# tudoroancea/ihm2

Measured on AMD Instinct MI355X. Metric: NMPC RTI solves/s (batch), N=40, nx=8 (6-DOF bicycle), fkin6, higher is better.
Workload: dtype f64

## Files before the change

ihm2_amd/csrc/kernels_qp.hip:

```cpp
#include <cstring>

#include "ihm2mpc_internal.h"
#include "device_steps.hpp"
#include "sqp_body.hpp"
#include "irk_body.hpp"
#include "riccati_mfma.hpp"
#include "sens_body.hpp"
#include "qp_lds.hpp"
#include "qp_mrows.hpp"
#include "qp_reduce.hpp"
#include "qp_div.hpp"
#include "qp_catalogue.hpp"
#include "wave_sync.hpp"

using namespace ihm2;

namespace {

#define INF_BOUND 1e20
#ifndef RIC_RING
#define RIC_RING 4
#endif
#ifndef SWEEP_RING
#define SWEEP_RING 4
#endif
#define SWEEP_DL ((SWEEP_RING >= 8) ? 4 : 2)

__device__ __forceinline__ bool fin(double v) { return fabs(v) < INF_BOUND; }
__device__ __forceinline__ int here(int v) { asm volatile("" : "+v"(v)); return v; }

template <typename OP>
__device__ __forceinline__ double wave_reduce(double v, OP op)
{
    v = op(v, dpp_mov<0xB1>(v));
    v = op(v, dpp_mov<0x4E>(v));
    v = op(v, dpp_mov<0x141>(v));
    v = op(v, dpp_mov<0x128>(v));
    int lo = __double2loint(v), hi = __double2hiint(v);
    auto a16 = __builtin_amdgcn_permlane16_swap(lo, lo, false, false);
    auto b16 = __builtin_amdgcn_permlane16_swap(hi, hi, false, false);
    v = op(__hiloint2double(b16[0], a16[0]), __hiloint2double(b16[1], a16[1]));
    lo = __double2loint(v); hi = __double2hiint(v);
    auto a32 = __builtin_amdgcn_permlane32_swap(lo, lo, false, false);
    auto b32 = __builtin_amdgcn_permlane32_swap(hi, hi, false, false);
    return op(__hiloint2double(b32[0], a32[0]), __hiloint2double(b32[1], a32[1]));
}
__device__ __forceinline__ double nanmax(double a, double b) { return (a != a || b != b) ? NAN : fmax(a, b); }
__device__ __forceinline__ double wave_max(double v) { return wave_reduce(v, [](double a, double b) { return fmax(a, b); }); }
__device__ __forceinline__ double wave_min(double v) { return wave_reduce(v, [](double a, double b) { return fmin(a, b); }); }
__device__ __forceinline__ double wave_sum(double v) { return wave_reduce(v, [](double a, double b) { return a + b; }); }
__device__ __forceinline__ double wave_nanmax(double v) { return wave_reduce(v, [](double a, double b) { return nanmax(a, b); }); }
__device__ __forceinline__ void norm_max(double &res, bool &bad, double v) { bad |= v != v; res = fmax(res, v); }

__device__ __forceinline__ double sum8(double v)
{
    v += dpp_mov<0xB1>(v);
    v += dpp_mov<0x4E>(v);
    v += dpp_mov<0x141>(v);
    return v;
}

// ... 128 lines not shown
#undef LEN
#define HS(k, i, l) (HL ? Hl[(((k) == N) ? 100 : 0) + (i) * 10 + (l)] : ((k) == N ? HsT : Hs0 + (UNI ? 0 : (k)) * 100)[(i) * 10 + (l)])
#define CDV(k, r, j) (CL ? CDl[(r) * 10 + (j)] : a.CD[((k) * 2 + (r)) * 10 + (j)])

    auto blk_reduce = [&](double v, auto op) -> double {
        v = wave_reduce(v, op);
        if (NW > 1) {
            __syncthreads();
            if (lane == 0) tile[wv] = v;
            __syncthreads();
            v = tile[0];
#pragma unroll
            for (int w = 1; w < NW; w++) v = op(v, tile[w]);
        }
        return v;
    };
    auto blk_max = [&](double v) { return blk_reduce(v, [](double x, double y) { return fmax(x, y); }); };
    auto blk_min = [&](double v) { return blk_reduce(v, [](double x, double y) { return fmin(x, y); }); };
    auto blk_sum = [&](double v) { return blk_reduce(v, [](double x, double y) { return x + y; }); };
    auto blk_nanmax = [&](double v) { return blk_reduce(v, [](double x, double y) { return nanmax(x, y); }); };

    const double *xb = a.x + (size_t)b * NS * 8;
    const double *ub = a.u + (size_t)b * N * 2;
    const double *linb = a.lin + (size_t)b * N * LIN_REC;
    double *gb = a.g + (size_t)b * NS * 10;
    double *rgb = a.rg + (size_t)b * NS * 10;
    double *Pg = a.P + (size_t)b * NS * 64;
    double *Mg = a.M + (size_t)b * N * 64;
    double *pib = a.pi + (size_t)b * NS * 8;
    double *lamb = a.lam + (size_t)b * NS * 28;
    double *slkb = a.slk + (size_t)b * NS * 28;
    double *lamab = ALAT ? a.lam_a + (size_t)b * NS * 2 : nullptr;
    double *slkab = ALAT ? a.slk_a + (size_t)b * NS * 2 : nullptr;
    auto alat_slot = [](int j) -> int { return (j == 3) ? 0 : (j == 4) ? 1 : (j == 6) ? 2 : (j == 7) ? 3 : -1; };

    if (HL) for (int e = tid; e < 200; e += NT) Hl[e] = (e < 100) ? Hs0[e] : HsT[e - 100];
    if (CL && tid < 20) CDl[tid] = a.CD[tid];
    if (UNI) BSYNC();
    bool h_sparse = false;
    if (HL) {
        int cnt = 0;
        if (tid < 20) {
#pragma unroll
            for (int l = 0; l < 10; l++) {
                const double v = Hl[tid * 10 + l];
                if (v != 0.0) { if (cnt < 3) { spv[tid * 3 + cnt] = v; spc[tid * 3 + cnt] = l; } cnt++; }
            }
            for (int q = cnt; q < 3; q++) { spv[tid * 3 + q] = 0.0; spc[tid * 3 + q] = 0; }
        }
        h_sparse = __ballot(cnt > 3) == 0ull;
        if (NW > 1) h_sparse = blk_max((wv == 0 && !h_sparse) ? 1.0 : 0.0) == 0.0;
        BSYNC();
    }
    double sg = 1.0, sb = 1.0, r_stat = 0.0, r_eq = 0.0;
    double w_R = 0.0, w_L = 0.0;
    if (PATH) {
        const int trk = a.track_id[b];
        w_R = a.widths[trk * 2 + 0]; w_L = a.widths[trk * 2 + 1];
        for (int k = tid; k < NS; k += NT) {
            const double psi = xb[k * 8 + 2], sgn = (psi > 0.0) - (psi < 0.0);
            const double dfoot = -0.5 * a.car_L * cos(fabs(psi)) * sgn, dlat = -0.5 * a.car_W * sin(psi);
            hc[k * 2 + 0] = (k >= 1) ? dfoot + dlat : 0.0;
            hc[k * 2 + 1] = (k >= 1) ? -dfoot + dlat : 0.0;
            if (ALAT) {
                double g4[4];
                alat_eval(xb[k * 8 + 3], xb[k * 8 + 4], xb[k * 8 + 6], xb[k * 8 + 7], g4);
#pragma unroll
                for (int q = 0; q < 4; q++) ha[k * 4 + q] = (k >= 1 && k < N) ? g4[q] : 0.0;
            }
        }
        BSYNC();
    }
    for (int e = tid; e < NS * 10; e += NT) {
        const int k = e / 10, j = e % 10;
        double acc = 0.0;
#pragma unroll
        for (int l = 0; l < 8; l++) acc = fma(HS(k, j, l), xb[k * 8 + l], acc);
        if (k < N) {
            acc = fma(HS(k, j, 8), ub[k * 2 + 0], acc);
            acc = fma(HS(k, j, 9), ub[k * 2 + 1], acc);
            const double *yr = a.yref + ((size_t)b * N + k) * 12;
#pragma unroll
            for (int l = 0; l < 12; l++) acc = fma(-Gy0[((UNI ? 0 : k) * 10 + j) * 12 + l], yr[l], acc);
        } else {
            const double *yr = a.yref_e + (size_t)b * 8;
#pragma unroll
            for (int l = 0; l < 8; l++) acc = fma(-GyT[j * 12 + l], yr[l], acc);
        }
        gb[e] = acc;
        const bool counted = !((k == 0 && j < 8) || (k == N && j >= 8));
        if (j < 8 || k < N) sg = fmax(sg, fabs(acc));
        if (!want_res) continue;
        double st = acc;
        if (k < N) {
            const double *rec = linb + (size_t)k * LIN_REC;
#pragma unroll
            for (int l = 0; l < 8; l++) st = fma((j < 8) ? rec[l * 8 + j] : rec[64 + l * 2 + (j - 8)], pib[(k + 1) * 8 + l], st);
        }
        if (j < 8) st -= pib[k * 8 + j];
        st -= lamb[k * 28 + j] - lamb[k * 28 + 14 + j];
        if (k < N) {
            st = fma(-CDV(k, 0, j), lamb[k * 28 + 10] - lamb[k * 28 + 24], st);
            st = fma(-CDV(k, 1, j), lamb[k * 28 + 11] - lamb[k * 28 + 25], st);
        }
        if (PATH && (j == 1 || j == 2)) {
            const double l12 = lamb[k * 28 + 12] - lamb[k * 28 + 26], l13 = lamb[k * 28 + 13] - lamb[k * 28 + 27];
// ... 68 lines not shown
            if (r < NSOFT) { const size_t po = (size_t)b * a.sl_bs + a.nslots_can; const double *zp = a.slot_lb + po, *Zp = a.slot_ub + po; so_zw[r < NSOFT ? r : 0] = zp[s]; so_Zw[r < NSOFT ? r : 0] = Zp[s]; soft = Zp[s] >= 0.0; }
#define LAM_IN(up) ((ALAT && c == 14) ? lamab[k * 2 + (up)] : lamb[k * 28 + 14 * (up) + c])
            if (fin(lb)) { s_dl[r] = lb - cz; if (want_res && !soft) { r_ineq = fmax(r_ineq, s_dl[r]); r_comp = fmax(r_comp, fabs(LAM_IN(0) * s_dl[r])); } }
            if (fin(ubd)) { s_du[r] = ubd - cz; if (want_res && !soft) { r_ineq = fmax(r_ineq, -s_du[r]); r_comp = fmax(r_comp, fabs(LAM_IN(1) * s_du[r])); } }
#undef LAM_IN
            if (ONE_SIDED(r) && fin(ubd)) { s_sg[r < NSOFT ? r : 0] = -1.0; s_dl[r] = -s_du[r]; }
        }
    }
    if (want_res) {
        if constexpr (FULL != 0) wave_max4(lane, r_stat, r_eq, r_ineq, r_comp);
        else { r_stat = blk_max(r_stat); r_eq = blk_max(r_eq); r_ineq = blk_max(r_ineq); r_comp = blk_max(r_comp); }
    }
    if (want_res && tid == 0) {
        double *rs = a.res + (size_t)b * 4;
        rs[0] = r_stat; rs[1] = r_eq; rs[2] = r_ineq; rs[3] = r_comp;
    }

    const double tol_g = a.tol * sg, tol_b = a.tol * sb, tol_d = a.tol * sb, tol_m = a.tol * sg;
    const double mu_floor = 0.1 * tol_m;
    const double mu0 = a.mu0 * sg;
    const double inv_m = (a.m_act > 0) ? 1.0 / a.m_act : 0.0;

    auto row_dot = [&](int kc, const double *v) -> double {
        const int k = kc / NCK, c = kc % NCK;
        if (c < 10) return v[k * 10 + c];
        if (ALAT && c == 14) return ha[k * 4] * v[k * 10 + 3] + ha[k * 4 + 1] * v[k * 10 + 4] + ha[k * 4 + 2] * v[k * 10 + 6] + ha[k * 4 + 3] * v[k * 10 + 7];
        if (PATH && c >= 12) return (c == 12) ? v[k * 10 + 1] + hc[k * 2] * v[k * 10 + 2] : -v[k * 10 + 1] + hc[k * 2 + 1] * v[k * 10 + 2];
        double acc = 0.0;
#pragma unroll
        for (int j = 0; j < 10; j++) acc = fma(CDV(k, c - 10, j), v[k * 10 + j], acc);
        return acc;
    };
    auto row_dot_full = [&](int r, const double *v) -> double {
        const int pk = here(s_kc[r]);
        return *reinterpret_cast<const double *>(reinterpret_cast<const char *>(pk < 0 ? tile : v) + ((pk >> 16) & 0x3fff));
    };
    static_assert(FULL == 0 || qp_general_rows_inside(qp_lds(NF > 0 ? NF : 2, CLS), NF > 0 ? NF : 2), "the general rows of a phase leave the transpose tile");
    auto general_rows = [&](const double *v) {
        for (int e0 = tid; e0 < 2 * N; e0 += 2 * NT) {
            const bool two = e0 + NT < 2 * N;
            const double *cd = CDl + (e0 & 1) * 10, *v0 = v + (e0 >> 1) * 10, *v1 = v + ((two ? e0 + NT : e0) >> 1) * 10;
            double c[10], p[10], q[10];
#pragma unroll
            for (int j = 0; j < 10; j++) { c[j] = cd[j]; p[j] = v0[j]; q[j] = v1[j]; }
            double acc0 = 0.0, acc1 = 0.0;
#pragma unroll
            for (int j = 0; j < 10; j++) { acc0 = fma(c[j], p[j], acc0); acc1 = fma(c[j], q[j], acc1); }
            tile[e0] = acc0;
            if (two) tile[e0 + NT] = acc1;
        }
        BSYNC();
    };

    for (int e = tid; e < NS * 10; e += NT) z[e] = (e < 8) ? a.x0[(size_t)b * 8 + e] - xb[e] : 0.0;
    for (int e = tid; e < NS * 8; e += NT) pi[e] = 0.0;
    if (FULL) for (int e = tid; e < NS * NCK; e += NT) { cf[e] = 0.0; gam[e] = 0.0; }
    BSYNC();
    if constexpr (FULL != 0) general_rows(z);
#pragma unroll
    for (int r = 0; r < NSLOT; r++) {
        if (NO_SLOT(r)) continue;
        const double rz = ROW_DOT(r, z);
        const bool al = HAS_L(r), au = HAS_U(r);
        double tau_c = a.tau0;
        if (al && au) tau_c = fmin(a.tau0, 0.25 * (s_du[r] - s_dl[r]));
        if (IS_SOFT(r)) {
            const double slack = al ? rz - s_dl[r] : s_du[r] - rz;
            const double s0 = fmax(a.tau0, a.tau0 - slack);
            so_s[r < NSOFT ? r : 0] = s0;
            so_ls[r < NSOFT ? r : 0] = mu0 / s0;
            if (al) { t_l[r] = slack + s0; lam_l[r] = mu0 / t_l[r]; } else { t_u[r] = slack + s0; lam_u[r] = mu0 / t_u[r]; }
            continue;
        }
        if (al) { t_l[r] = fmax(rz - s_dl[r], tau_c); lam_l[r] = mu0 / t_l[r]; }
        if (au) { t_u[r] = fmax(s_du[r] - rz, tau_c); lam_u[r] = mu0 / t_u[r]; }
    }

    int qstatus = 1, it = 0;
    bool exact_mode = false;
    double res_g = 0, res_b = 0, res_d = 0, res_m = 0, mu = 0;
    double fol_g = 0.0, fol_b = 0.0;
    double rd_l[NSLOT], rd_u[NSLOT], dlam_l[NSLOT], dlam_u[NSLOT], dt_l[NSLOT], dt_u[NSLOT];
    double pa_l[NSLOT], pa_u[NSLOT];
    for (it = 0;; it++) {
        bool exact = (it == 0) || exact_mode, finished = false;
        auto multipliers_to_cf = [&]() {
            if (!FULL) {
                for (int e = tid; e < NS * NCK; e += NT) cf[e] = 0.0;
                BSYNC();
            }
#pragma unroll
            for (int r = 0; r < NSLOT; r++) {
                if (NO_SLOT(r)) continue;
                const bool al = HAS_L(r), au = HAS_U(r);
                SLOT_ACC(SLOT_AT(cf, r), ROW_SIGN(r, (al ? lam_l[r] : 0.0) - (au ? lam_u[r] : 0.0)));
            }
            BSYNC();
        };
        if (LEAN != 0) { if (exact) multipliers_to_cf(); }
        else {
            for (int e = tid; e < NS * NCK; e += NT) cf[e] = 0.0;
            BSYNC();
        }
        double mu_acc = 0.0, res_gs = 0.0;
        res_d = 0.0; res_m = 0.0;
        double lane_d = 0.0, lane_m = 0.0;
        bool bad_d = false, bad_m = false, bad_gs = false;
        if constexpr (FULL != 0) general_rows(z);
#pragma unroll
        for (int r = 0; r < NSLOT; r++) {
            rd_l[r] = rd_u[r] = 0.0;
            if (NO_SLOT(r)) continue;
            const double rz = ROW_DOT(r, z);
            const bool al = HAS_L(r), au = HAS_U(r);
            const double sv = IS_SOFT(r) ? so_s[r < NSOFT ? r : 0] : 0.0;
            double pl = 0.0, pu = 0.0;
            if constexpr (FULL != 0) {
                rd_l[r] = rz - t_l[r] - s_dl[r] + sv; pl = __dmul_rn(lam_l[r], t_l[r]); norm_max(lane_m, bad_m, fabs(pl));
                rd_u[r] = s_du[r] - rz - t_u[r] + sv; pu = __dmul_rn(lam_u[r], t_u[r]); norm_max(lane_m, bad_m, fabs(pu));
            } else {
            if (al) { rd_l[r] = rz - t_l[r] - s_dl[r] + sv; pl = __dmul_rn(lam_l[r], t_l[r]); res_m = nanmax(res_m, fabs(pl)); }
            if (au) { rd_u[r] = s_du[r] - rz - t_u[r] + sv; pu = __dmul_rn(lam_u[r], t_u[r]); res_m = nanmax(res_m, fabs(pu)); }
            }
            mu_acc = __dadd_rn(mu_acc, __dadd_rn(pl, pu));
            if constexpr (FULL != 0) { bad_d |= __builtin_isunordered(rd_l[r], rd_u[r]); lane_d = fmax(lane_d, fmax(fabs(rd_l[r]), fabs(rd_u[r]))); }
            else
            res_d = nanmax(res_d, nanmax(fabs(rd_l[r]), fabs(rd_u[r])));
            if (IS_SOFT(r)) {
                const int q = r < NSOFT ? r : 0;
                so_rs[q] = so_Zw[q] * so_s[q] + so_zw[q] - (al ? lam_l[r] : lam_u[r]) - so_ls[q];
                if constexpr (FULL != 0) {
                    norm_max(res_gs, bad_gs, fabs(so_rs[q]));
                    mu_acc += so_ls[q] * so_s[q]; norm_max(lane_m, bad_m, fabs(so_ls[q] * so_s[q]));
                } else {
                res_gs = nanmax(res_gs, fabs(so_rs[q]));
                mu_acc += so_ls[q] * so_s[q]; res_m = nanmax(res_m, fabs(so_ls[q] * so_s[q]));
                }
            }
            if (LEAN == 0) SLOT_ACC(SLOT_AT(cf, r), ROW_SIGN(r, (al ? lam_l[r] : 0.0) - (au ? lam_u[r] : 0.0)));
        }
        if constexpr (NW > 1) {
#pragma unroll
            for (int r = 0; r < NSLOT; r++) {
                const int sidx = tid + NT * r;
                if (sidx >= a.nslots_can) continue;
                const bool on = s_kc[r] >= 0;
                gam[sidx] = __dadd_rn((on && fin(s_dl[r])) ? __dmul_rn(lam_l[r], t_l[r]) : 0.0, (on && fin(s_du[r])) ? __dmul_rn(lam_u[r], t_u[r]) : 0.0);
            }
            __syncthreads();
            mu_acc = 0.0;
            for (int sidx = lane; sidx < a.nslots_can; sidx += 64) mu_acc = __dadd_rn(mu_acc, gam[sidx]);
            __syncthreads();
        }
        if (LEAN == 0) BSYNC();
        for (int rpass = 0; rpass < 2; rpass++) {
            if (exact) {
                for (int e = tid; e < NS * 10; e += NT) {
                    const int k = e / 10, j = e % 10;
                    double acc = gb[e];
                    if (HL && h_sparse) {
                        const int row = ((k == N) ? 10 : 0) + j;
#pragma unroll
                        for (int q = 0; q < 3; q++) acc = fma(spv[row * 3 + q], z[k * 10 + spc[row * 3 + q]], acc);
                    } else {
#pragma unroll
                        for (int l = 0; l < 10; l++) acc = fma(HS(k, j, l), z[k * 10 + l], acc);
                    }
                    if (k < N) {
                        acc = fma(-CDV(k, 0, j), cf[k * NCK + 10], acc);
                        acc = fma(-CDV(k, 1, j), cf[k * NCK + 11], acc);
                    }
                    if (j < 8) acc -= pi[k * 8 + j];
                    acc -= cf[k * NCK + j];
                    if (PATH && (j == 1 || j == 2)) {
                        const double l12 = cf[k * NCK + 12], l13 = cf[k * NCK + 13];
                        acc -= (j == 1) ? l12 - l13 : hc[k * 2] * l12 + hc[k * 2 + 1] * l13;
                    }
                    if (ALAT && alat_slot(j) >= 0) acc -= ha[k * 4 + alat_slot(j)] * cf[k * NCK + 14];
                    gt[e] = acc;
                }
                BSYNC();
                dyn_residual<4, NT>(N, tid, const_cast<double *>(linb), z, pi, gt, rb, LIN_REC);
                BSYNC();
            }
            res_g = 0.0; res_b = 0.0;
            if (exact || LEAN == 0) {
                for (int e = tid; e < NS * 10; e += NT) {
                    const int k = e / 10, j = e % 10;
                    double v = gt[e];
                    if ((k == 0 && j < 8) || (k == N && j >= 8)) { v = 0.0; gt[e] = 0.0; }
                    if (exact) rgb[e] = v;
                    res_g = nanmax(res_g, fabs(v));
                }
                for (int e = tid; e < N * 8; e += NT) res_b = nanmax(res_b, fabs(rb[e]));
            } else { res_g = fol_g; res_b = fol_b; }
            if constexpr (FULL != 0) {
                const bool nan_g = wave_any(res_g != res_g || bad_gs), nan_b = wave_any(res_b != res_b), nan_d = wave_any(bad_d), nan_m = wave_any(bad_m);
                res_g = fmax(res_g, res_gs);
                res_d = lane_d; res_m = lane_m;
                wave_max4(lane, res_g, res_b, res_d, res_m);
                mu = wave_sum(mu_acc) * inv_m;
                res_g = nan_g ? NAN : res_g; res_b = nan_b ? NAN : res_b; res_d = nan_d ? NAN : res_d; res_m = nan_m ? NAN : res_m;
            } else {
            res_g = nanmax(res_g, res_gs);
            res_g = blk_nanmax(res_g); res_b = blk_nanmax(res_b);
            if (rpass == 0) { res_d = blk_nanmax(res_d); res_m = blk_nanmax(res_m); mu = ((NW == 1) ? blk_sum(mu_acc) : wave_sum(mu_acc)) * inv_m; }
            }
            if (!(res_g == res_g) || !(res_b == res_b) || !(res_d == res_d) || !(res_m == res_m)) { qstatus = (it == 0) ? 3 : 4; finished = true; break; }
            const bool conv = res_g <= tol_g && res_b <= tol_b && res_d <= tol_d && res_m <= tol_m;
            if (conv && exact) { qstatus = 0; finished = true; break; }
            if ((conv || it >= a.iter_max) && !exact) {
                exact = true; exact_mode = true;
                if (LEAN != 0) multipliers_to_cf();
                continue;
            }
            break;
        }
        if (finished) break;
        if (it >= a.iter_max) { qstatus = 1; break; }
        BSYNC();
        double alpha = 1.0, alpha_d = 1.0, sigma = 0.0;
        auto slot_coeffs = [&](int pass) {
            if (!FULL) {
                for (int e = tid; e < NS * NCK; e += NT) { cf[e] = 0.0; if (pass == 0) gam[e] = 0.0; }
                BSYNC();
            }
            const double mu_t = fmax(sigma * mu, mu_floor);
            if constexpr (FULL != 0) {
                if (pass == 1) {
                    double cn[2 * NSLOT], cd[2 * NSLOT], cq[2 * NSLOT];
#pragma unroll
                    for (int r = 0; r < NSLOT; r++) { cn[2 * r] = pa_l[r] - mu_t; cd[2 * r] = t_l[r]; cn[2 * r + 1] = pa_u[r] - mu_t; cd[2 * r + 1] = t_u[r]; }
                    div_sets<DIVW_COEFF>(cn, cd, cq);
#pragma unroll
                    for (int r = 0; r < NSLOT; r++) {
                        double c = 0.0;
                        c += cq[2 * r];
                        c -= cq[2 * r + 1];
                        SLOT_AT(cf, r) = c;
// ... 28 lines not shown
                    if (au) c -= (pa_u[r] - mu_t) / t_u[r];
                }
                SLOT_ACC(SLOT_AT(cf, r), ROW_SIGN(r, c));
            }
            BSYNC();
        };
        auto add_coeffs = [&]() {
            for (int e = tid; e < NS * 10; e += NT) {
                const int k = e / 10, j = e % 10;
                double acc = gt[e] + cf[k * NCK + j];
                if (k < N) {
                    acc = fma(CDV(k, 0, j), cf[k * NCK + 10], acc);
                    acc = fma(CDV(k, 1, j), cf[k * NCK + 11], acc);
                }
                if (PATH && (j == 1 || j == 2)) {
                    const double c12 = cf[k * NCK + 12], c13 = cf[k * NCK + 13];
                    acc += (j == 1) ? c12 - c13 : hc[k * 2] * c12 + hc[k * 2 + 1] * c13;
                }
                if (ALAT && alat_slot(j) >= 0) acc += ha[k * 4 + alat_slot(j)] * cf[k * NCK + 14];
                gt[e] = acc;
            }
            BSYNC();

        };
        slot_coeffs(0);
        add_coeffs();
        __builtin_amdgcn_s_waitcnt(0x0F70);
        if (wv == 0) {
            RicLds L;
            const QpRic o = qp_lds_ric(N, NS, NCK);
            L.gt = o.gt; L.pv = o.pv; L.gam = o.gam; L.dz = o.dz; L.kff = o.kff; L.Kl = o.Kl;
            L.Ginv = o.Ginv; L.hv = o.Prb; L.tile = o.tile; L.hc = o.hc; L.ha = o.ha;
            if constexpr (NF != 0)
                riccati_sweep_mfma<NCK, PATH != 0, UNI != 0, RIC_RING, ALAT, true, (NF > 0) ? NF : 0>(N, lane, linb, Hs0, HsT, a.CD, L, Pg, Mg, LIN_REC, false, false);
            else
            riccati_sweep_mfma<NCK, PATH != 0, UNI != 0, RIC_RING, ALAT>(N, lane, linb, Hs0, HsT, a.CD, L, Pg, Mg, LIN_REC, a.m_act == 0, a.symmetrize != 0);
            if (lane < 8) dz[lane] = 0.0;
        }
        BSYNC();
        double it_l[NSLOT], it_u[NSLOT];
        if constexpr (FULL != 0) {
            double one[2 * NSLOT], tt[2 * NSLOT], rc[2 * NSLOT];
#pragma unroll
            for (int r = 0; r < NSLOT; r++) { one[2 * r] = one[2 * r + 1] = 1.0; tt[2 * r] = t_l[r]; tt[2 * r + 1] = t_u[r]; }
            div_sets<DIVW_RECIP>(one, tt, rc);
#pragma unroll
            for (int r = 0; r < NSLOT; r++) { it_l[r] = rc[2 * r]; it_u[r] = rc[2 * r + 1]; }
        }
        for (int pass = 0; pass < 2; pass++) {
            const double mu_t = fmax(sigma * mu, mu_floor);
            if (pass == 1) slot_coeffs(1);
            if (pass == 1) {
            add_coeffs();
            for (int e = tid; e < NS * 8; e += NT) {
                const int k = e >> 3, j = e & 7;
                double v = gt[k * 10 + j];
                if (k < N) v -= Kl[k * 16 + j] * gt[k * 10 + 8] + Kl[k * 16 + 8 + j] * gt[k * 10 + 9];
                pv[e] = v;
            }
            BSYNC();
            if constexpr (LEAN != 0) {
            if (wv == 0) {
                const int g = lane >> 3, w = lane & 7;
                double pw = pv[N * 8 + w], pg = 0.0;
                const int se2 = (w == 0) ? 16 : 0, so2 = (g == 0) ? 16 : 0;
                const double *be = (w == 0) ? pv + (N - 1) * 8 + g : dz, *bo = (g == 0) ? pv + (N - 2) * 8 + w : dz;
                const double *qe = Prb + (N - 1) * 8 + w, *qo = Prb + (N - 2) * 8 + g;
                double *oe = pv + (N - 1) * 8 + g, *oo = pv + (N - 2) * 8 + w;
                stream_rows<-1, SWEEP_RING, SWEEP_DL, true, PAIRM>(Mg, N, RIC_IDX(w, g), RIC_IDX(g, w),
                    [&](int k, bool odd, double &prb, double &base) {
                        if (odd) { prb = *qo; qo -= 16; base = *bo; bo -= so2; } else { prb = *qe; qe -= 16; base = *be; be -= se2; }
                    },
                    [&](int k, double m, bool odd, double prb, double base) {
                        if (!odd) {
                            pg = sum8(fma(m, pw, fma(m, prb, base)));
                            *oe = pg; oe -= 16;
                        } else {
                            pw = sum_stride8(fma(m, pg, fma(m, prb, base)));
                            *oo = pw; oo -= 16;
                        }
                    });
            }
            } else {
            if (wv == 0) {
                const int g = lane >> 3, w = lane & 7;
                double pw = pv[N * 8 + w], pg = 0.0;
                stream_rows_v1<-1, QP_V1_RING, QP_V1_DL>(Mg, N, RIC_IDX(w, g), RIC_IDX(g, w),
                    [&](int k, bool odd, double &prb, double &base) { prb = Prb[k * 8 + (odd ? g : w)]; base = pv[k * 8 + (odd ? w : g)]; },
                    [&](int k, double m, bool odd, double prb, double base) {
                        if (!odd) {
                            const double off = fma(m, prb, (w == 0) ? base : 0.0);
                            pg = sum8(fma(m, pw, off));
                            if (w == 0) pv[k * 8 + g] = pg;
                        } else {
                            const double off = fma(m, prb, (g == 0) ? base : 0.0);
                            pw = sum_stride8(fma(m, pg, off));
                            if (g == 0) pv[k * 8 + w] = pw;
                        }
                    });
            }
            }
            BSYNC();
            for (int k = tid; k < N; k += NT) {
                const double *rec = linb + (size_t)k * LIN_REC;
                double g0 = gt[k * 10 + 8], g1 = gt[k * 10 + 9];
                double Bk[16];
#pragma unroll
                for (int l = 0; l < 16; l++) Bk[l] = rec[64 + l];
#pragma unroll
                for (int l = 0; l < 8; l++) {
                    const double h = Prb[k * 8 + l] + pv[(k + 1) * 8 + l];
                    g0 = fma(Bk[l * 2 + 0], h, g0);
                    g1 = fma(Bk[l * 2 + 1], h, g1);
                }
                const double kf0 = Ginv[k * 8 + 0] * g0 + Ginv[k * 8 + 1] * g1;
                const double kf1 = Ginv[k * 8 + 1] * g0 + Ginv[k * 8 + 2] * g1;
                kff[k * 4 + 0] = kf0;
                kff[k * 4 + 1] = kf1;
#pragma unroll
                for (int i = 0; i < 8; i++) dz[(k + 1) * 10 + i] = rb[k * 8 + i] - Bk[i * 2] * kf0 - Bk[i * 2 + 1] * kf1;
            }
            if (tid < 8) dz[tid] = 0.0;
            BSYNC();
            }

            if constexpr (LEAN != 0) {
            if (wv == 0) {
                const int g = lane >> 3, w = lane & 7;
                double dxw = dz[w], dxg = 0.0;
                const int se2 = (w == 0) ? 20 : 0, so2 = (g == 0) ? 20 : 0;
                const double *ce = (w == 0) ? dz + 10 + g : dz, *co = (g == 0) ? dz + 20 + w : dz;
                stream_rows<+1, SWEEP_RING, SWEEP_DL, true, PAIRM>(Mg, N, RIC_IDX(g, w), RIC_IDX(w, g),
                    [&](int k, bool odd, double &c, double &unused) {
                        if (odd) { c = *co; co += so2; } else { c = *ce; ce += se2; }
                        unused = 0.0;
                    },
                    [&](int k, double m, bool odd, double c, double) {
                        if (!odd) {
                            dxg = sum8(fma(m, dxw, c));
                            dz[(k + 1) * 10 + g] = dxg;
                        } else {
                            dxw = sum_stride8(fma(m, dxg, c));
                            dz[(k + 1) * 10 + w] = dxw;
                        }
                    });
            }
            } else {
            if (wv == 0) {
                const int g = lane >> 3, w = lane & 7;
                double dxw = dz[w], dxg = 0.0;
                stream_rows_v1<+1, QP_V1_RING, QP_V1_DL>(Mg, N, RIC_IDX(g, w), RIC_IDX(w, g),
                    [&](int k, bool odd, double &c, double &unused) { c = dz[(k + 1) * 10 + (odd ? w : g)]; unused = 0.0; },
                    [&](int k, double m, bool odd, double c, double) {
                        if (!odd) {
                            dxg = sum8(fma(m, dxw, (w == 0) ? c : 0.0));
                            if (w == 0) dz[(k + 1) * 10 + g] = dxg;
                        } else {
                            dxw = sum_stride8(fma(m, dxg, (g == 0) ? c : 0.0));
                            if (g == 0) dz[(k + 1) * 10 + w] = dxw;
                        }
                    });
            }
            }
            BSYNC();
            const bool want_dpi = (pass == 1) || (a.m_act == 0);
            for (int e = tid; e < NS * 2; e += NT) {
                const int k = e >> 1, aa = e & 1;
                double acc = 0.0;
                if (k < N) {
                    acc = -kff[k * 4 + aa];
#pragma unroll
                    for (int l = 0; l < 8; l++) acc = fma(-Kl[k * 16 + aa * 8 + l], dz[k * 10 + l], acc);
                }
                dz[k * 10 + 8 + aa] = acc;
            }
            if (want_dpi) {
                const int n = NS * 8;
                for (int base = 0; base < n; base += 3 * NT) {
                    double2 pr[3][4];
#pragma unroll
                    for (int q = 0; q < 3; q++) {
                        const int e = min(base + NT * q + tid, n - 1), k = e >> 3, i = e & 7;
#pragma unroll
                        for (int l = 0; l < 4; l++) pr[q][l] = *reinterpret_cast<const double2 *>(Pg + (size_t)k * 64 + RIC_IDX(l, i));
                    }
#pragma unroll
                    for (int q = 0; q < 3; q++) {
                        const int e = base + NT * q + tid, ec = min(e, n - 1), k = ec >> 3;
                        double acc = pv[ec];
#pragma unroll
                        for (int l = 0; l < 4; l++) { acc = fma(pr[q][l].x, dz[k * 10 + l], acc); acc = fma(pr[q][l].y, dz[k * 10 + l + 4], acc); }
                        if (e < n) pv[e] = acc;
                    }
                }
            }
            BSYNC();

            double amax = 1.0, amax_d = 1.0, mu_aff = 0.0, rmax = 1.0, rmax_d = 1.0;
            if constexpr (FULL != 0) general_rows(dz);
            if constexpr (FULL != 0) {
                double drz[NSLOT], qn[2 * NSLOT], qd[2 * NSLOT], qq[2 * NSLOT];
#pragma unroll
                for (int r = 0; r < NSLOT; r++) drz[r] = ROW_DOT(r, dz);
#pragma unroll
                for (int r = 0; r < NSLOT; r++) {
                    {
                        const double rm = (pass == 0) ? lam_l[r] * t_l[r] : lam_l[r] * t_l[r] + pa_l[r] - mu_t;
                        dt_l[r] = drz[r] + rd_l[r];
                        dlam_l[r] = -(rm + lam_l[r] * dt_l[r]) * it_l[r];
                    }
                    {
                        const double rm = (pass == 0) ? lam_u[r] * t_u[r] : lam_u[r] * t_u[r] + pa_u[r] - mu_t;
                        dt_u[r] = -drz[r] + rd_u[r];
                        dlam_u[r] = -(rm + lam_u[r] * dt_u[r]) * it_u[r];
                    }
                    qn[2 * r] = -dlam_l[r]; qd[2 * r] = lam_l[r]; qn[2 * r + 1] = -dlam_u[r]; qd[2 * r + 1] = lam_u[r];
                }
                div_sets<DIVW_STEP>(qn, qd, qq);
// ... 61 lines not shown
                }
            }
            if constexpr (FULL != 0) {
                const double one[2] = {1.0, 1.0}, rm2[2] = {rmax, rmax_d};
                double rc[2];
                div_batch<2>(one, rm2, rc);
                amax = fmin(amax, rc[0]); amax_d = fmin(amax_d, rc[1]);
            } else
            if (NSOFT == 0) { amax = fmin(amax, 1.0 / rmax); amax_d = fmin(amax_d, 1.0 / rmax_d); }
            if constexpr (FULL != 0) wave_min2(lane, amax, amax_d);
            else { amax = blk_min(amax); amax_d = blk_min(amax_d); }
            if (pass == 0) {
                if (a.m_act == 0) { alpha = alpha_d = 1.0; break; }
#pragma unroll
                for (int r = 0; r < NSLOT; r++) {
                    pa_l[r] = dlam_l[r] * dt_l[r]; pa_u[r] = dlam_u[r] * dt_u[r];
                    if (NO_SLOT(r)) continue;
                    mu_aff = __dadd_rn(mu_aff, __dadd_rn(HAS_L(r) ? __dmul_rn(fma(amax_d, dlam_l[r], lam_l[r]), fma(amax, dt_l[r], t_l[r])) : 0.0,
                                                         HAS_U(r) ? __dmul_rn(fma(amax_d, dlam_u[r], lam_u[r]), fma(amax, dt_u[r], t_u[r])) : 0.0));
                    if (IS_SOFT(r)) {
                        const int q = r < NSOFT ? r : 0;
                        so_pa[q] = so_dls[q] * so_ds[q];
                        mu_aff += (so_ls[q] + amax_d * so_dls[q]) * (so_s[q] + amax * so_ds[q]);
                    }
                }
                if constexpr (NW > 1) {
#pragma unroll
                    for (int r = 0; r < NSLOT; r++) {
                        const int sidx = tid + NT * r;
                        if (sidx >= a.nslots_can) continue;
                        const bool on = s_kc[r] >= 0;
                        gam[sidx] = __dadd_rn((on && fin(s_dl[r])) ? __dmul_rn(fma(amax_d, dlam_l[r], lam_l[r]), fma(amax, dt_l[r], t_l[r])) : 0.0,
                                              (on && fin(s_du[r])) ? __dmul_rn(fma(amax_d, dlam_u[r], lam_u[r]), fma(amax, dt_u[r], t_u[r])) : 0.0);
                    }
                    __syncthreads();
                    mu_aff = 0.0;
                    for (int sidx = lane; sidx < a.nslots_can; sidx += 64) mu_aff = __dadd_rn(mu_aff, gam[sidx]);
                    __syncthreads();
                    mu_aff = wave_sum(mu_aff) * inv_m;
                } else
                mu_aff = blk_sum(mu_aff) * inv_m;
                const double ratio = (mu > 0.0) ? mu_aff / mu : 0.0;
                sigma = ratio * ratio * ratio;
            } else {
                alpha = fmin(1.0, IHM2MPC_IPM_STEP_FRACTION * amax); alpha_d = fmin(1.0, IHM2MPC_IPM_STEP_FRACTION * amax_d);
            }
            BSYNC();
        }
        if (fmin(alpha, alpha_d) < 1e-12) { qstatus = 2; break; }
        if (!exact_mode) {
            const double cd = 1.0 - alpha_d, cp = alpha - alpha_d, cb = 1.0 - alpha;
            const int n10 = NS * 10;
            fol_g = 0.0; fol_b = 0.0;
            for (int base = 0; base < n10; base += 4 * NT) {
                double ro[4];
#pragma unroll
                for (int q = 0; q < 4; q++) ro[q] = rgb[min(base + NT * q + tid, n10 - 1)];
#pragma unroll
                for (int q = 0; q < 4; q++) {
                    const int e = base + NT * q + tid, ec = min(e, n10 - 1), k = ec / 10, j = ec % 10;
                    double hdz = 0.0;
                    if (HL && h_sparse) {
                        const int row = ((k == N) ? 10 : 0) + j;
#pragma unroll
                        for (int l = 0; l < 3; l++) hdz = fma(spv[row * 3 + l], dz[k * 10 + spc[row * 3 + l]], hdz);
                    } else {
#pragma unroll
                        for (int l = 0; l < 10; l++) hdz = fma(HS(k, j, l), dz[k * 10 + l], hdz);
                    }
                    const bool masked = (k == 0 && j < 8) || (k == N && j >= 8);
                    const double v = masked ? 0.0 : fma(cp, hdz, cd * ro[q]);
                    if (e < n10) { rgb[e] = v; gt[e] = v; if (LEAN != 0) fol_g = nanmax(fol_g, fabs(v)); }
                }
            }
            for (int e = tid; e < N * 8; e += NT) {
                const double v = cb * rb[e];
                rb[e] = v;
                if (LEAN != 0) fol_b = nanmax(fol_b, fabs(v));
                const_cast<double *>(linb)[(size_t)(e >> 3) * LIN_REC + RIC_REC_RB + (e & 7)] = v;
            }
        }
        for (int e = tid; e < NS * 10; e += NT) z[e] = fma(alpha, dz[e], z[e]);
        for (int e = tid; e < NS * 8; e += NT) pi[e] = fma(alpha_d, pv[e], pi[e]);
#pragma unroll
        for (int r = 0; r < NSLOT; r++) {
            if (NO_SLOT(r)) continue;
            if (HAS_L(r)) { lam_l[r] = fma(alpha_d, dlam_l[r], lam_l[r]); t_l[r] = fma(alpha, dt_l[r], t_l[r]); }
            if (HAS_U(r)) { lam_u[r] = fma(alpha_d, dlam_u[r], lam_u[r]); t_u[r] = fma(alpha, dt_u[r], t_u[r]); }
            if (IS_SOFT(r)) { const int q = r < NSOFT ? r : 0; so_s[q] = fma(alpha, so_ds[q], so_s[q]); so_ls[q] = fma(alpha_d, so_dls[q], so_ls[q]); }
        }
        BSYNC();
    }
    if (qstatus == 1 && !(res_g <= 1e4 * tol_g && res_b <= 1e4 * tol_b && res_d <= 1e4 * tol_d && res_m <= 1e4 * tol_m)) qstatus = 4;

    int st = 0;
    if (qstatus == 3) st = 1;
    else if (qstatus == 2 || qstatus == 4) st = 4;
    BSYNC();
    if (st == 0) {
        double bad = 0.0;
        for (int e = tid; e < NS * 10; e += NT) bad = fmax(bad, isfinite(z[e]) ? 0.0 : 1.0);
        if (blk_max(bad) > 0.0) st = 1;
    }
    double *xw = a.x + (size_t)b * NS * 8, *uw = a.u + (size_t)b * N * 2;
    if (NSOFT > 0) {
        for (int e = tid; e < NS * 28; e += NT) slkb[e] = 0.0;
        if (ALAT) for (int e = tid; e < NS * 2; e += NT) slkab[e] = 0.0;
    }
    if (st == 0) {
        for (int e = tid; e < NS * 10; e += NT) {
            const int k = e / 10, j = e % 10;
            if (j < 8) xw[k * 8 + j] += z[e];
            else if (k < N) uw[k * 2 + j - 8] += z[e];
        }
        for (int e = tid; e < NS * 8; e += NT) pib[e] = (e < 8) ? 0.0 : pi[e];
        for (int e = tid; e < NS * 28; e += NT) lamb[e] = 0.0;
        if (ALAT) for (int e = tid; e < NS * 2; e += NT) lamab[e] = 0.0;
        __syncthreads();
#pragma unroll
        for (int r = 0; r < NSLOT; r++) {
            if (NO_SLOT(r)) continue;
            const int k = SLOT_W(r) / NCK, c = SLOT_W(r) % NCK;
            if (ONE_SIDED(r)) {
                const int up = (s_sg[r < NSOFT ? r : 0] < 0.0) ? 1 : 0;
                if (ALAT && c == 14) { lamab[k * 2 + up] = lam_l[r]; if (IS_SOFT(r)) slkab[k * 2 + up] = so_s[r < NSOFT ? r : 0]; }
                else { lamb[k * 28 + 14 * up + c] = lam_l[r]; if (IS_SOFT(r)) slkb[k * 28 + 14 * up + c] = so_s[r < NSOFT ? r : 0]; }
                continue;
            }
            if (ALAT && c == 14) {
                if (fin(s_dl[r])) lamab[k * 2] = lam_l[r];
                if (fin(s_du[r])) lamab[k * 2 + 1] = lam_u[r];
                if (IS_SOFT(r)) slkab[k * 2 + (fin(s_dl[r]) ? 0 : 1)] = so_s[r < NSOFT ? r : 0];
                continue;
            }
            if (fin(s_dl[r])) lamb[k * 28 + c] = lam_l[r];
            if (fin(s_du[r])) lamb[k * 28 + 14 + c] = lam_u[r];
            if (IS_SOFT(r)) slkb[k * 28 + (fin(s_dl[r]) ? c : 14 + c)] = so_s[r < NSOFT ? r : 0];
        }
    }
    __syncthreads();
    if (tid < 2) a.u0[(size_t)b * 2 + tid] = uw[tid];
    if (tid == 0) {
        a.status[b] = st; a.qp_iter[b] = it;
        double *q = a.qp_res + (size_t)b * 4;
        q[0] = res_g / tol_g * a.tol; q[1] = res_b / tol_b * a.tol; q[2] = res_d / tol_d * a.tol; q[3] = res_m / tol_m * a.tol;
    }
}

#undef BSYNC

template <int NSLOT, int NSOFT, int PATH, int UNI, int NF = 0, int FULL = 0>
__global__ __launch_bounds__(64) void k_qp_wave(QpArgs a)
{
    extern __shared__ double sm[];
    if ((int)blockIdx.x >= a.B) return;
    if (NF > 0 && a.N != NF) return;
    qp_wave_body<NSLOT, NSOFT, PATH, UNI, 1, 1, NF, FULL>(a, blockIdx.x, sm);
}

template <int NSLOT, int UNI, int NW>
__global__ __launch_bounds__(64 * NW) void k_qp_block(QpArgs a)
{
// ... 221 lines not shown
```

Measured before the change: 1.386 million.

## Map QP vector passes to column-per-lane layout with register-held Hessian rows

```diff
diff --git a/ihm2_amd/csrc/kernels_qp.hip b/ihm2_amd/csrc/kernels_qp.hip
--- a/ihm2_amd/csrc/kernels_qp.hip
+++ b/ihm2_amd/csrc/kernels_qp.hip
@@ -7,6 +7,7 @@
 #include "riccati_mfma.hpp"
 #include "sens_body.hpp"
 #include "qp_lds.hpp"
+#include "qp_lanecols.hpp"
 #include "qp_mrows.hpp"
 #include "qp_reduce.hpp"
 #include "qp_div.hpp"
@@ -241,6 +242,25 @@
         if (NW > 1) h_sparse = blk_max((wv == 0 && !h_sparse) ? 1.0 : 0.0) == 0.0;
         BSYNC();
     }
+    static_assert(FULL == 0 || (HL && qlc_reads_inside(qp_lds(NF > 0 ? NF : 2, CLS), (NF > 0 ? NF : 2) + 1, 4)), "the column-per-lane passes: H in LDS, reads inside the block");
+    [[maybe_unused]] const int LC_ROUNDS = qlc_rounds(NS), LC_TERM = qlc_term_round(N);
+    [[maybe_unused]] auto lc_lane = [&]() -> LcLane { const int l = here(lane); return {qlc_col(l), qlc_sub(l), qlc_active(l), qlc_sub(l) == qlc_term_sub(N)}; };
+    [[maybe_unused]] auto lc_load = [&](auto &row, const LcLane &lc) { row.load(Hl, spv, spc, lc.j); };
+    [[maybe_unused]] auto lc_dot = [&](auto &row, const LcLane &lc, int r, const double *vk, double acc) -> double {
+        if (r == LC_TERM) row.terminal(Hl, lc.j, lc.term);
+        return row.dot(vk, acc);
+    };
+    constexpr int BATCH_WORDS = 4 * NT * 2;
+    static_assert(FULL == 0 || qp_lds(NF > 0 ? NF : 2, CLS).dz + BATCH_WORDS <= qp_lds(NF > 0 ? NF : 2, CLS).total, "the batched in-place updates read past the block's LDS (dz is the last array they read)");
+    [[maybe_unused]] auto axpy_batched = [&](double *y, const double *x, const double al, const int n) {
+        for (int base = tid; base < n; base += 4 * NT) {
+            double yo[4], xo[4];
+#pragma unroll
+            for (int q = 0; q < 4; q++) { yo[q] = y[base + NT * q]; xo[q] = x[base + NT * q]; }
+#pragma unroll
+            for (int q = 0; q < 4; q++) if (base + NT * q < n) y[base + NT * q] = fma(al, xo[q], yo[q]);
+        }
+    };
     double sg = 1.0, sb = 1.0, r_stat = 0.0, r_eq = 0.0;
     double w_R = 0.0, w_L = 0.0;
     if (PATH) {
@@ -415,6 +435,13 @@
         BSYNC();
     };
 
+    if constexpr (FULL != 0) {
+        const LcLane lc = lc_lane();
+        for (int r = 0; r < LC_ROUNDS; r++) {
+            const int e = lane + QLC_LANES * r;
+            if (lc.on && e < NS * 10) z[e] = (e < 8) ? a.x0[(size_t)b * 8 + e] - xb[e] : 0.0;
+        }
+    } else
     for (int e = tid; e < NS * 10; e += NT) z[e] = (e < 8) ? a.x0[(size_t)b * 8 + e] - xb[e] : 0.0;
     for (int e = tid; e < NS * 8; e += NT) pi[e] = 0.0;
     if (FULL) for (int e = tid; e < NS * NCK; e += NT) { cf[e] = 0.0; gam[e] = 0.0; }
@@ -518,6 +545,26 @@
         if (LEAN == 0) BSYNC();
         for (int rpass = 0; rpass < 2; rpass++) {
             if (exact) {
+                if constexpr (FULL != 0) {
+                    const LcLane lc = lc_lane();
+                    const double cd0 = CDl[lc.j], cd1 = CDl[10 + lc.j];
+                    auto rounds = [&](auto &&row_dot_h) {
+                        for (int r = 0; r < LC_ROUNDS; r++) {
+                            const int e = lane + QLC_LANES * r, k = QLC_STAGES * r + lc.sub;
+                            double acc = gb[min(e, NS * 10 - 1)];
+                            acc = row_dot_h(r, z + k * 10, acc);
+                            if (k < N) {
+                                acc = fma(-cd0, cf[k * NCK + 10], acc);
+                                acc = fma(-cd1, cf[k * NCK + 11], acc);
+                            }
+                            if (lc.j < 8) acc -= pi[k * 8 + lc.j];
+                            acc -= cf[k * NCK + lc.j];
+                            if (lc.on && e < NS * 10) gt[e] = acc;
+                        }
+                    };
+                    if (h_sparse) { LcSparseRow row; lc_load(row, lc); rounds([&](int r, const double *vk, double acc) { return lc_dot(row, lc, r, vk, acc); }); }
+                    else { LcDenseRow row; lc_load(row, lc); rounds([&](int r, const double *vk, double acc) { return lc_dot(row, lc, r, vk, acc); }); }
+                } else
                 for (int e = tid; e < NS * 10; e += NT) {
                     const int k = e / 10, j = e % 10;
                     double acc = gb[e];
@@ -548,6 +595,18 @@
             }
             res_g = 0.0; res_b = 0.0;
             if (exact || LEAN == 0) {
+                if constexpr (FULL != 0) {
+                    const LcLane lc = lc_lane();
+                    for (int r = 0; r < LC_ROUNDS; r++) {
+                        const int e = lane + QLC_LANES * r, k = QLC_STAGES * r + lc.sub;
+                        if (lc.on && e < NS * 10) {
+                            double v = gt[e];
+                            if ((k == 0 && lc.j < 8) || (k == N && lc.j >= 8)) { v = 0.0; gt[e] = 0.0; }
+                            if (exact) rgb[e] = v;
+                            res_g = nanmax(res_g, fabs(v));
+                        }
+                    }
+                } else
                 for (int e = tid; e < NS * 10; e += NT) {
                     const int k = e / 10, j = e % 10;
                     double v = gt[e];
@@ -682,6 +741,25 @@
             if (pass == 1) slot_coeffs(1);
             if (pass == 1) {
             add_coeffs();
+            if constexpr (FULL != 0) {
+                static_assert(qp_lds(NF, CLS).Kl + ((NF + 1) * 8 + 3 * 64 - 1) / (3 * 64) * (3 * 64) / 8 * 16 <= qp_lds(NF, CLS).total, "the corrector's base term reads K past the block's LDS");
+                for (int base = tid; base < NS * 8; base += 3 * NT) {
+                    double g[3], g8[3], g9[3], k0[3], k1[3];
+#pragma unroll
+                    for (int q = 0; q < 3; q++) {
+                        const int e = base + NT * q, k = e >> 3, j = e & 7;
+                        g[q] = gt[k * 10 + j]; g8[q] = gt[k * 10 + 8]; g9[q] = gt[k * 10 + 9];
+                        k0[q] = Kl[k * 16 + j]; k1[q] = Kl[k * 16 + 8 + j];
+                    }
+#pragma unroll
+                    for (int q = 0; q < 3; q++) {
+                        const int e = base + NT * q, k = e >> 3;
+                        double v = g[q];
+                        if (k < N) v = __dsub_rn(v, fma(k0[q], g8[q], __dmul_rn(k1[q], g9[q])));
+                        if (e < NS * 8) pv[e] = v;
+                    }
+                }
+            } else
             for (int e = tid; e < NS * 8; e += NT) {
                 const int k = e >> 3, j = e & 7;
                 double v = gt[k * 10 + j];
@@ -731,6 +809,38 @@
             }
             }
             BSYNC();
+            if constexpr (FULL != 0) {
+                static_assert(LIN_REC % 2 == 0, "the records' B_k on 16-byte boundaries");
+                for (int k = tid; k < N; k += NT) {
+                    const double2 *B2 = reinterpret_cast<const double2 *>(linb + (size_t)k * LIN_REC + 64);
+                    const double2 *P2 = reinterpret_cast<const double2 *>(Prb + k * 8), *V2 = reinterpret_cast<const double2 *>(pv + (k + 1) * 8);
+                    const double2 *R2 = reinterpret_cast<const double2 *>(rb + k * 8);
+                    double g0 = gt[k * 10 + 8], g1 = gt[k * 10 + 9];
+                    double2 Bk[8], rbk[4];
+#pragma unroll
+                    for (int l = 0; l < 8; l++) Bk[l] = B2[l];
+#pragma unroll
+                    for (int l = 0; l < 4; l++) rbk[l] = R2[l];
+#pragma unroll
+                    for (int l = 0; l < 4; l++) {
+                        const double2 p = P2[l], v = V2[l];
+                        const double h0 = p.x + v.x, h1 = p.y + v.y;
+                        g0 = fma(Bk[2 * l].x, h0, g0);
+                        g1 = fma(Bk[2 * l].y, h0, g1);
+                        g0 = fma(Bk[2 * l + 1].x, h1, g0);
+                        g1 = fma(Bk[2 * l + 1].y, h1, g1);
+                    }
+                    const double2 gi = *reinterpret_cast<const double2 *>(Ginv + k * 8);
+                    const double gi2 = Ginv[k * 8 + 2];
+                    const double kf0 = gi.x * g0 + gi.y * g1;
+                    const double kf1 = gi.y * g0 + gi2 * g1;
+                    *reinterpret_cast<double2 *>(kff + k * 4) = make_double2(kf0, kf1);
+                    double2 *D2 = reinterpret_cast<double2 *>(dz + (k + 1) * 10);
+#pragma unroll
+                    for (int l = 0; l < 4; l++)
+                        D2[l] = make_double2(rbk[l].x - Bk[2 * l].x * kf0 - Bk[2 * l].y * kf1, rbk[l].y - Bk[2 * l + 1].x * kf0 - Bk[2 * l + 1].y * kf1);
+                }
+            } else
             for (int k = tid; k < N; k += NT) {
                 const double *rec = linb + (size_t)k * LIN_REC;
                 double g0 = gt[k * 10 + 8], g1 = gt[k * 10 + 9];
@@ -794,6 +904,27 @@
             }
             BSYNC();
             const bool want_dpi = (pass == 1) || (a.m_act == 0);
+            if constexpr (FULL != 0) {
+                static_assert(NF + 1 <= 64, "one lane per stage");
+                if (tid < NS) {
+                    const int k = tid;
+                    double a0 = 0.0, a1 = 0.0;
+                    if (k < N) {
+                        const double2 *D2 = reinterpret_cast<const double2 *>(dz + k * 10), *K2 = reinterpret_cast<const double2 *>(Kl + k * 16);
+                        const double2 kf = *reinterpret_cast<const double2 *>(kff + k * 4);
+                        double2 d[4], k0[4], k1[4];
+#pragma unroll
+                        for (int l = 0; l < 4; l++) { d[l] = D2[l]; k0[l] = K2[l]; k1[l] = K2[4 + l]; }
+                        a0 = -kf.x; a1 = -kf.y;
+#pragma unroll
+                        for (int l = 0; l < 4; l++) {
+                            a0 = fma(-k0[l].x, d[l].x, a0); a1 = fma(-k1[l].x, d[l].x, a1);
+                            a0 = fma(-k0[l].y, d[l].y, a0); a1 = fma(-k1[l].y, d[l].y, a1);
+                        }
+                    }
+                    *reinterpret_cast<double2 *>(dz + k * 10 + 8) = make_double2(a0, a1);
+                }
+            } else
             for (int e = tid; e < NS * 2; e += NT) {
                 const int k = e >> 1, aa = e & 1;
                 double acc = 0.0;
@@ -961,6 +1092,26 @@
             const double cd = 1.0 - alpha_d, cp = alpha - alpha_d, cb = 1.0 - alpha;
             const int n10 = NS * 10;
             fol_g = 0.0; fol_b = 0.0;
+            if constexpr (FULL != 0) {
+                const LcLane lc = lc_lane();
+                auto rounds = [&](auto &&row_dot_h) {
+                    for (int r0 = 0; r0 < LC_ROUNDS; r0 += 4) {
+                        double ro[4];
+#pragma unroll
+                        for (int q = 0; q < 4; q++) ro[q] = rgb[min(lane + QLC_LANES * (r0 + q), n10 - 1)];
+#pragma unroll
+                        for (int q = 0; q < 4; q++) {
+                            const int r = r0 + q, e = lane + QLC_LANES * r, k10 = e - lc.j;
+                            const double hdz = row_dot_h(r, dz + k10, 0.0);
+                            const bool masked = (k10 == 0 && lc.j < 8) || (k10 == N * 10 && lc.j >= 8);
+                            const double v = masked ? 0.0 : fma(cp, hdz, cd * ro[q]);
+                            if (lc.on && e < n10) { rgb[e] = v; gt[e] = v; fol_g = nanmax(fol_g, fabs(v)); }
+                        }
+                    }
+                };
+                if (h_sparse) { LcSparseRow row; lc_load(row, lc); rounds([&](int r, const double *vk, double acc) { return lc_dot(row, lc, r, vk, acc); }); }
+                else { LcDenseRow row; lc_load(row, lc); rounds([&](int r, const double *vk, double acc) { return lc_dot(row, lc, r, vk, acc); }); }
+            } else
             for (int base = 0; base < n10; base += 4 * NT) {
                 double ro[4];
 #pragma unroll
@@ -982,6 +1133,23 @@
                     if (e < n10) { rgb[e] = v; gt[e] = v; if (LEAN != 0) fol_g = nanmax(fol_g, fabs(v)); }
                 }
             }
+            if constexpr (FULL != 0) {
+                for (int base = tid; base < N * 8; base += 4 * NT) {
+                    double o[4];
+#pragma unroll
+                    for (int q = 0; q < 4; q++) o[q] = rb[base + NT * q];
+#pragma unroll
+                    for (int q = 0; q < 4; q++) {
+                        const int e = base + NT * q;
+                        const double v = cb * o[q];
+                        if (e < N * 8) {
+                            rb[e] = v;
+                            fol_b = nanmax(fol_b, fabs(v));
+                            const_cast<double *>(linb)[(size_t)(e >> 3) * LIN_REC + RIC_REC_RB + (e & 7)] = v;
+                        }
+                    }
+                }
+            } else
             for (int e = tid; e < N * 8; e += NT) {
                 const double v = cb * rb[e];
                 rb[e] = v;
@@ -989,8 +1157,11 @@
                 const_cast<double *>(linb)[(size_t)(e >> 3) * LIN_REC + RIC_REC_RB + (e & 7)] = v;
             }
         }
+        if constexpr (FULL != 0) { axpy_batched(z, dz, alpha, NS * 10); axpy_batched(pi, pv, alpha_d, NS * 8); }
+        else {
         for (int e = tid; e < NS * 10; e += NT) z[e] = fma(alpha, dz[e], z[e]);
         for (int e = tid; e < NS * 8; e += NT) pi[e] = fma(alpha_d, pv[e], pi[e]);
+        }
 #pragma unroll
         for (int r = 0; r < NSLOT; r++) {
             if (NO_SLOT(r)) continue;
@@ -1017,6 +1188,27 @@
         if (ALAT) for (int e = tid; e < NS * 2; e += NT) slkab[e] = 0.0;
     }
     if (st == 0) {
+        if constexpr (FULL != 0) {
+            const LcLane lc = lc_lane();
+            double *const wp = (lc.j < 8) ? xw + lc.sub * 8 + lc.j : uw + lc.sub * 2 + (lc.j - 8);
+            const int ws = (lc.j < 8) ? QLC_STAGES * 8 : QLC_STAGES * 2;
+            for (int r0 = 0; r0 < LC_ROUNDS; r0 += 4) {
+                double o[4], dzv[4];
+#pragma unroll
+                for (int q = 0; q < 4; q++) {
+                    const int r = r0 + q, k = QLC_STAGES * r + lc.sub;
+                    const bool own = lc.on && k <= N && (lc.j < 8 || k < N);
+                    o[q] = own ? wp[r * ws] : 0.0;
+                    dzv[q] = z[lane + QLC_LANES * r];
+                }
+#pragma unroll
+                for (int q = 0; q < 4; q++) {
+                    const int r = r0 + q, k = QLC_STAGES * r + lc.sub;
+                    const bool own = lc.on && k <= N && (lc.j < 8 || k < N);
+                    if (own) wp[r * ws] = o[q] + dzv[q];
+                }
+            }
+        } else
         for (int e = tid; e < NS * 10; e += NT) {
             const int k = e / 10, j = e % 10;
             if (j < 8) xw[k * 8 + j] += z[e];
diff --git a/ihm2_amd/csrc/qp_lanecols.hpp b/ihm2_amd/csrc/qp_lanecols.hpp
--- /dev/null
+++ b/ihm2_amd/csrc/qp_lanecols.hpp
@@ -0,0 +1,80 @@
+#pragma once
+
+#include <cmath>
+
+#include "qp_lds.hpp"
+
+#ifdef __HIPCC__
+#define QLC_HD __host__ __device__ __forceinline__
+#define QLC_UNROLL _Pragma("unroll")
+#else
+#define QLC_HD inline
+#define QLC_UNROLL
+#endif
+
+namespace ihm2 {
+
+constexpr int QLC_COLS = 10, QLC_STAGES = 6, QLC_LANES = QLC_COLS * QLC_STAGES;
+
+QP_LDS_FN bool qlc_active(int lane) { return lane >= 0 && lane < QLC_LANES; }
+QP_LDS_FN int qlc_col(int lane) { return lane % QLC_COLS; }
+QP_LDS_FN int qlc_sub(int lane) { return lane / QLC_COLS; }
+QP_LDS_FN int qlc_stage(int lane, int r) { return QLC_STAGES * r + qlc_sub(lane); }
+QP_LDS_FN int qlc_elem(int lane, int r) { return lane + QLC_LANES * r; }
+QP_LDS_FN bool qlc_owns(int lane, int r, int NS) { return qlc_active(lane) && r >= 0 && qlc_elem(lane, r) < NS * QLC_COLS; }
+QP_LDS_FN int qlc_rounds(int NS) { return (NS * QLC_COLS + QLC_LANES - 1) / QLC_LANES; }
+QP_LDS_FN int qlc_term_round(int N) { return N / QLC_STAGES; }
+QP_LDS_FN int qlc_term_sub(int N) { return N % QLC_STAGES; }
+struct LcLane { int j, sub; bool on, term; };
+QP_LDS_FN int qlc_read_end(int rounds) { return (QLC_STAGES * rounds + 1) * QLC_COLS; }
+QP_LDS_FN int qlc_batched_rounds(int NS, int depth) { return (qlc_rounds(NS) + depth - 1) / depth * depth; }
+QP_LDS_FN bool qlc_reads_inside(const QpLds &l, int NS, int depth)
+{
+    const int end = qlc_read_end(qlc_batched_rounds(NS, depth));
+    return l.z + end <= l.total && l.gt + end <= l.total && l.dz + end <= l.total && l.cf + end / QLC_COLS * (l.cf.len / NS) <= l.total;
+}
+
+static_assert(qlc_rounds(41) == 7 && qlc_term_round(40) == 6 && qlc_term_sub(40) == 4 && qlc_stage(49, 6) == 40 && qlc_elem(49, 6) == 409, "N = 40: seven rounds, stage 40 in the lanes 40..49 of the last");
+static_assert(qlc_reads_inside(qp_lds(40, qp_lds_class(0, true)), 41, 4) && qlc_reads_inside(qp_lds(2, qp_lds_class(0, true)), 3, 4), "a pass's unclamped reads leave the LDS");
+
+struct LcSparseRow {
+    double v[3], tv[3];
+    int c[3], tc[3];
+    QLC_HD void load(const double *, const double *spv, const int *spc, int j)
+    {
+        QLC_UNROLL
+        for (int l = 0; l < 3; l++) { v[l] = spv[j * 3 + l]; c[l] = spc[j * 3 + l]; tv[l] = spv[30 + j * 3 + l]; tc[l] = spc[30 + j * 3 + l]; }
+    }
+    QLC_HD void terminal(const double *, int, bool mine)
+    {
+        QLC_UNROLL
+        for (int l = 0; l < 3; l++) { v[l] = mine ? tv[l] : v[l]; c[l] = mine ? tc[l] : c[l]; }
+    }
+    QLC_HD double dot(const double *vk, double acc) const
+    {
+        QLC_UNROLL
+        for (int l = 0; l < 3; l++) acc = fma(v[l], vk[c[l]], acc);
+        return acc;
+    }
+};
+struct LcDenseRow {
+    double v[10];
+    QLC_HD void load(const double *Hl, const double *, const int *, int j)
+    {
+        QLC_UNROLL
+        for (int l = 0; l < 10; l++) v[l] = Hl[j * 10 + l];
+    }
+    QLC_HD void terminal(const double *Hl, int j, bool mine)
+    {
+        QLC_UNROLL
+        for (int l = 0; l < 10; l++) v[l] = Hl[(mine ? 100 : 0) + j * 10 + l];
+    }
+    QLC_HD double dot(const double *vk, double acc) const
+    {
+        QLC_UNROLL
+        for (int l = 0; l < 10; l++) acc = fma(v[l], vk[l], acc);
+        return acc;
+    }
+};
+
+}
```

Result: no change. 1.380 million (-0.4%).
